# kyumcu/firedancer

Measured on AMD Instinct MI355X. Metric: Ed25519 verifies/sec, higher is better.
Workload: dtype u32

## Files before the change

firedancer_amd/csrc/fd_curve25519_dev.h:

```cpp

#ifndef FD_CURVE25519_DEV_H
#define FD_CURVE25519_DEV_H

#include "fd_f25519_dev.h"

#if defined(__HIPCC__)
#define FD_GE_FN __device__ __forceinline__
#else
#define FD_GE_FN static
#endif

struct ge_p3     { fe X, Y, Z, T; };
struct ge_cached { fe YpX, YmX, T2d, Z2; };
struct ge_precomp{ fe YpX, YmX, T2d; };

FD_FN void fe_const_d( fe & r ) {
  r.v[0]=0x35978a3u; r.v[1]=0x0d37284u; r.v[2]=0x3156ebdu; r.v[3]=0x06a0a0eu; r.v[4]=0x001c029u;
  r.v[5]=0x179e898u; r.v[6]=0x3a03cbbu; r.v[7]=0x1ce7198u; r.v[8]=0x2e2b6ffu; r.v[9]=0x1480db3u;
}
FD_FN void fe_const_d2( fe & r ) {
  r.v[0]=0x2b2f159u; r.v[1]=0x1a6e509u; r.v[2]=0x22add7au; r.v[3]=0x0d4141du; r.v[4]=0x0038052u;
  r.v[5]=0x0f3d130u; r.v[6]=0x3407977u; r.v[7]=0x19ce331u; r.v[8]=0x1c56dffu; r.v[9]=0x0901b67u;
}
FD_FN void fe_const_sqrtm1( fe & r ) {
// ... 70 lines not shown
  fe_mul( TT, p.T, q.T2d );
  FE_FENCE();
  fe_add( D, p.Z, p.Z );
  fe_sub( E, PP, MM );
  fe_add( H, PP, MM );
  fe_add( G, D, TT );
  fe_sub( F, D, TT );
  fe_mul( r.X, F, E );
  FE_FENCE();
  fe_mul( r.Y, H, G );
  FE_FENCE();
  fe_mul( r.Z, F, G );
  FE_FENCE();
  if( want_t ) fe_mul( r.T, H, E );
  FE_FENCE();
}

FD_FN void ge_to_cached( ge_cached & c, ge_p3 const & p ) {
  fe d2; fe_const_d2( d2 );
  fe_add( c.YpX, p.Y, p.X );
  fe_sub( c.YmX, p.Y, p.X );
  fe_mul( c.T2d, p.T, d2 );
  FE_FENCE();
  fe_add( c.Z2, p.Z, p.Z );
}

FD_FN void ge_from_cached( ge_p3 & r, ge_cached const & c ) {
  fe t;
  t.v[0] = c.YpX.v[0] + FE_4P0 - c.YmX.v[0];
#pragma unroll
// ... 118 lines not shown
```

firedancer_amd/csrc/fd_diag.h:

```cpp

#ifndef FD_DIAG_H
#define FD_DIAG_H

#if !defined(FD_DIAG_BUILD)
#if defined(FD_DIAG_NO_VTAB_STORE) || defined(FD_DIAG_VTAB_ONE_ENTRY) || defined(FD_DIAG_VTAB_NO_TAIL) || \
    defined(FD_DIAG_SC_TABLES) || defined(FD_DIAG_NT_TABLES) || defined(FD_DIAG_NT_INV) ||                 \
    defined(FD_DIAG_SC_INV_AFTER) || defined(FD_DIAG_COMB_POS) || defined(FD_DIAG_LSORT_TIMEOUT) ||         \
    defined(FD_DIAG_PIPE_OVERLAP) || defined(FD_DIAG_NO_HAND) || defined(FD_DIAG_NO_ARENA) || defined(FD_DIAG_STORE_COAL) || \
    defined(FD_DIAG_STORE_SMALL) || defined(FD_DIAG_STORE_COAL_NT)
#error "FD_DIAG_* builds a wrong-results diagnostic variant: only tools/build_var.sh (FD_DIAG_BUILD) may define one"
#endif
#endif


#define FD_VTAB_TAIL        1
#define FD_COMB_POS_RUN     FD_CTAB_POS
#define FD_LSORT_SPIN       (1u << 20)
#define FD_DIAG_VTAB_STORE( m, tl, w )   do {} while( 0 )
#define FD_DIAG_FETCH_ENTRY( e )         do {} while( 0 )
#define FD_DIAG_PHASE_BC_ENTRY()         do {} while( 0 )
#define FD_DIAG_AFTER_TABLES()           do {} while( 0 )
#define FD_DIAG_SCR_ORDER                1
#define FD_DIAG_NO_HAND_ON               0
#define FD_DIAG_NO_ARENA_ON              0

#if defined(__HIPCC__)
__device__ __forceinline__ uint32_t fd_diag_bp_word( int j ) { return j ? 0x66666666u : 0x66666658u; }
__device__ __forceinline__ uint32_t fd_diag_hash( uint64_t g, uint32_t j ) {
  uint32_t x = (uint32_t)g * 0x9e3779b1u ^ (j + 1u) * 0x85ebca6bu;
  x ^= x >> 15; x *= 0x2c1b3c6du; x ^= x >> 12; x *= 0x297a2d39u; x ^= x >> 15;
  return x;
}
#endif

#if defined(FD_DIAG_BUILD)

#if defined(FD_DIAG_VTAB_NO_TAIL)
#undef  FD_VTAB_TAIL
#define FD_VTAB_TAIL 0
// ... 10 lines not shown
#endif

#if defined(FD_DIAG_PIPE_OVERLAP)
#undef  FD_DIAG_SCR_ORDER
#define FD_DIAG_SCR_ORDER 0
#endif

#if defined(FD_DIAG_NO_HAND)
#undef  FD_DIAG_NO_HAND_ON
#define FD_DIAG_NO_HAND_ON 1
#endif

#if defined(FD_DIAG_NO_ARENA)
#undef  FD_DIAG_NO_ARENA_ON
#define FD_DIAG_NO_ARENA_ON 1
#endif

#if defined(FD_DIAG_VTAB_ONE_ENTRY)
#undef  FD_DIAG_FETCH_ENTRY
#define FD_DIAG_FETCH_ENTRY( e ) do { (e) = 0u; } while( 0 )
#endif

#if defined(FD_DIAG_NO_VTAB_STORE)
#undef  FD_DIAG_VTAB_STORE
#define FD_DIAG_VTAB_STORE( m, tl, w ) do {                                                       \
    if( (w)[0] == 0xdeadbeefu && (w)[1] == 0xdeadbeefu ) (m)[0] = make_uint4( (w)[2], (w)[3], (w)[4], (w)[5] ); \
    return; } while( 0 )
#elif defined(FD_DIAG_STORE_COAL)
#undef  FD_DIAG_VTAB_STORE
#define FD_DIAG_VTAB_STORE( m, tl, w ) do {                                                       \
// ... 68 lines not shown
```

firedancer_amd/csrc/fd_ed25519_gpu_host.cpp:

```cpp

#include <hip/hip_runtime_api.h>
#include <dlfcn.h>
#include <stdlib.h>
#include <string.h>
#include <stdio.h>
#include <time.h>
#include <condition_variable>
#include <functional>
#include <thread>
#include <mutex>
#include <string>
#include <unordered_map>
#include <vector>

#include "fd_ed25519_gpu_abi.h"
#include "fd_diag.h"

static uint64_t align_up( uint64_t x, uint64_t a ) { return (x + a - 1u) / a * a; }

static unsigned char const fd_ed25519_gpu_hsaco[] = {
#include "fd_ed25519_gpu_hsaco.inc"
};
#include "fd_build_id.h"

// ... 909 lines not shown
    if( s->phand[k] ) hipFree( s->phand[k] );
    if( s->pst[k] )   hipFree( s->pst[k] );
    if( s->pnw[k] )   hipFree( s->pnw[k] );
    s->phand[k] = NULL; s->pst[k] = NULL; s->pnw[k] = NULL;
  }
  for( int k=0; k<2; k++ ) {
    if( s->pacc[k] )  hipFree( s->pacc[k] );
    if( s->pcode[k] ) hipFree( s->pcode[k] );
    s->pacc[k] = NULL; s->pcode[k] = NULL;
  }
  if( s->perr ) hipHostFree( s->perr );
  s->pvtab = NULL; s->perr = NULL; s->d_perr = NULL;
  s->pipe_ready = 0;
}

static int
pipe_reserve( fd_dev_state * s ) {
  if( s->pipe_ready ) return FD_ED25519_GPU_OK;
  HIPCK( hipSetDevice( s->dev ) );
  pipe_free( s );
  uint64_t cap = s->sig_cap;
  uint64_t words = (uint64_t)FD_VTAB_N * FD_VTAB_WORDS * (2u * FD_PIPE_SETS * cap);
  int err = FD_ED25519_GPU_OK;
  if( fd_gpu_test_fail_alloc() || hipMalloc( &s->pvtab, (words + FD_VTAB_WORDS) * sizeof(uint32_t) ) != hipSuccess ) {
    s->pvtab = NULL; err = FD_ED25519_GPU_ERR_OOM;
  }
  for( int k=0; k<FD_PIPE_SETS && !err; k++ ) {
    if( hipMalloc( &s->phand[k], (uint64_t)FD_PH_WORDS * cap * sizeof(uint32_t) ) != hipSuccess ) { s->phand[k] = NULL; err = FD_ED25519_GPU_ERR_OOM; break; }
    if( hipMalloc( &s->pst[k], cap ) != hipSuccess )               { s->pst[k] = NULL; err = FD_ED25519_GPU_ERR_OOM; break; }
    if( hipMalloc( &s->pnw[k], cap / 64u + 1u ) != hipSuccess )    { s->pnw[k] = NULL; err = FD_ED25519_GPU_ERR_OOM; break; }
// ... 2 lines not shown
    if( fd_gpu_test_fail_alloc() ||
        hipMalloc( &s->pacc[k], (uint64_t)FD_PACC_WORDS * cap * sizeof(uint32_t) ) != hipSuccess ) { s->pacc[k] = NULL; err = FD_ED25519_GPU_ERR_OOM; break; }
    if( hipMalloc( &s->pcode[k], cap ) != hipSuccess ) { s->pcode[k] = NULL; err = FD_ED25519_GPU_ERR_OOM; break; }
  }
  if( !err && (hipHostMalloc( (void **)&s->perr, FD_PIPE_ERR_RING * sizeof(uint32_t), hipHostMallocMapped ) != hipSuccess ||
               hipHostGetDevicePointer( (void **)&s->d_perr, s->perr, 0 ) != hipSuccess) ) {
    if( s->perr ) hipHostFree( s->perr );
    s->perr = NULL; s->d_perr = NULL; err = FD_ED25519_GPU_ERR_OOM;
  }
  if( !err ) {
    for( int k=0; k<FD_PIPE_ERR_RING; k++ ) ((volatile uint32_t *)s->perr)[ k ] = 0u;
    err = vtab_id_fill( s, s->pvtab, 2u * FD_PIPE_SETS * cap );
  }
  if( err ) { pipe_free( s ); return err; }
  s->pctr = 0; s->pb[0].n = 0; s->pb[1].n = 0; s->pb[0].tag = -1; s->pb[1].tag = -1;
  char const * e = getenv( "FD_ED25519_GPU_PIPE_KB" );
  long kb = e ? atol( e ) : 8;
  s->pkb = kb < 1 ? 1u : (uint64_t)kb;
  e = getenv( "FD_ED25519_GPU_PIPE_LSORT" );
  s->plsort = !(e && e[0] == '0');
  e = getenv( "FD_ED25519_GPU_PIPE_PRIO" );
  s->pprio = 0;
  if( e && strlen( e ) == 3 )
    for( int k=0; k<3; k++ ) s->pprio |= (uint64_t)((e[k] - '0') & 3) << (2*k);
  s->pipe_ready = 1;
  return FD_ED25519_GPU_OK;
}

static int
pipe_launch( fd_ed25519_gpu_t * ctx, fd_dev_state * s, uint8_t const * d_arena, uint64_t arena_sz,
             fd_ed25519_desc_t const * d_desc, uint64_t n, uint32_t const * d_ncnt, int8_t * d_out, int tag,
             hipStream_t st, int * done_tag, uint32_t const * kpre = NULL, fparse_args const * fp = NULL ) {
  pipe_args a;
  memset( &a, 0, sizeof(a) );
// ... 115 lines not shown
  int err2 = scr_release( s, st );
  return err ? err : err2;
}

int
fd_ed25519_gpu_pipe_flush_dev( fd_ed25519_gpu_t * ctx, int dev_idx, void * stream ) {
  if( !ctx || dev_idx < 0 || dev_idx >= ctx->ndev ) return FD_ED25519_GPU_ERR_ARG;
  fd_dev_state * s = &ctx->d[ dev_idx ];
  if( !s->pipe_ready ) return FD_ED25519_GPU_OK;
  if( ctx->aq_cnt || ctx->fq_cnt ) return FD_ED25519_GPU_ERR_BUSY;
  for( int k=0; k<2 && pipe_busy( s ); k++ ) {
    int err = fd_ed25519_gpu_pipe_dev( ctx, dev_idx, NULL, 0u, NULL, 0u, NULL, stream );
    if( err ) return err;
  }
  return FD_ED25519_GPU_OK;
}

int
fd_ed25519_gpu_pipe_status( fd_ed25519_gpu_t * ctx, int dev_idx ) {
  if( !ctx || dev_idx < 0 || dev_idx >= ctx->ndev ) return FD_ED25519_GPU_ERR_ARG;
  return pipe_err_take( &ctx->d[ dev_idx ] );
}


static int
aslot_reserve( fd_dev_state * s, fd_dev_state::aslot * e, uint64_t span_sz, uint64_t m ) {
  if( !e->copied ) {
    if( hipEventCreateWithFlags( &e->copied, s->evflags ) != hipSuccess ) { e->copied = NULL; return FD_ED25519_GPU_ERR_LAUNCH; }
    if( hipEventCreateWithFlags( &e->done, s->doneflags ) != hipSuccess ) {
      hipEventDestroy( e->copied ); e->copied = NULL; e->done = NULL; return FD_ED25519_GPU_ERR_LAUNCH;
// ... 1059 lines not shown
```

firedancer_amd/csrc/fd_ed25519_gpu_kern.hip:

```cpp

#include <hip/hip_runtime.h>

#include "fd_ed25519_gpu_abi.h"
#include "fd_f25519_dev.h"
#include "fd_curve25519_dev.h"
#include "fd_sha512_dev.h"
#include "fd_sha256_dev.h"
#include "fd_scalar_dev.h"
#include "fd_lattice_dev.h"
#include "fd_diag.h"

#ifndef FD_OPT_FIRSTWIN
#define FD_OPT_FIRSTWIN 1
#endif
#ifndef FD_OPT_COMBCHK
#define FD_OPT_COMBCHK 1
#endif
#ifndef FD_OPT_IDROW
#define FD_OPT_IDROW 2
#endif
#ifndef FD_OPT_TAIL1
#define FD_OPT_TAIL1 1
#endif
#ifndef FD_OPT_APARSE
#define FD_OPT_APARSE 1
#endif
#ifndef FD_OPT_APRIO
#define FD_OPT_APRIO 1
#endif
#ifndef FD_OPT_BNOT
#define FD_OPT_BNOT 1
#endif
#ifndef FD_OPT_X4
#define FD_OPT_X4 1
#endif

#ifdef FD_PHASE_STAMPS
#define FD_NSTAMP 8
#define FD_TL_BASE 8
#define FD_STAMP_WORDS_DEV (8u + 4096u * 12u * 4u)
#define STAMP( i ) do { FE_FENCE(); if( _st ) _st[ i ] = __builtin_amdgcn_s_memtime(); FE_FENCE(); } while( 0 )
#else
#define STAMP( i ) do {} while( 0 )
#endif


typedef unsigned int fd_u4a4 __attribute__(( ext_vector_type( 4 ), aligned( 4 ) ));

template<int M>
// ... 204 lines not shown
      int k = 4*j + i;
      w[i] = (k == FD_VW( 0, 0 ) || k == FD_VW( 1, 0 )) ? 1u : (k == FD_VW( 3, 0 ) ? 2u : 0u);
    }
    m[j] = make_uint4( w[0], w[1], w[2], w[3] );
  }
  tl[0] = make_uint4( 0u, 0u, 0u, 0u ); tl[1] = make_uint4( 0u, 0u, 0u, 0u );
}

__device__ __forceinline__ uint32_t vtab_entry( uint32_t db ) {
  uint32_t e;
  asm( "v_sad_u32 %0, %1, 8, 0" : "=v"(e) : "v"(db) );
  return min( e, 8u );
}

__device__ __forceinline__ void vtab_store( uint32_t * vtab, uint64_t cap, uint64_t t, int e, ge_cached const & c,
                                            bool tail = true ) {
  uint32_t w[ 40 ];
#pragma unroll
  for( int j=0; j<10; j++ ) {
    w[FD_VW(0,j)] = c.YpX.v[j]; w[FD_VW(1,j)] = c.YmX.v[j]; w[FD_VW(2,j)] = c.T2d.v[j]; w[FD_VW(3,j)] = c.Z2.v[j];
  }
  uint4 const * mc; uint4 const * tc;
  vtab_ptrs( vtab, cap, t, (uint32_t)e, &mc, &tc );
  uint4 * m = (uint4 *)mc; uint4 * tl = (uint4 *)tc;
  FD_DIAG_VTAB_STORE( m, tl, w );
#pragma unroll
  for( int j=0; j<8; j++ ) m[j] = make_uint4( w[4*j], w[4*j+1], w[4*j+2], w[4*j+3] );
#if FD_VTAB_TAIL
  if( tail ) {
#pragma unroll
    for( int j=0; j<2; j++ ) tl[j] = make_uint4( w[32+4*j], w[33+4*j], w[34+4*j], w[35+4*j] );
  }
#endif
}

__device__ __forceinline__ void vtab_build( uint32_t * vtab, uint64_t cap, uint64_t t, ge_p3 const & Q ) {
  ge_p3 nQ = Q;
  { fe x; fe_neg( x, Q.X ); fe_carry( nQ.X, x ); fe_neg( x, Q.T ); fe_carry( nQ.T, x ); }
  ge_cached c;
// ... 149 lines not shown
#ifdef FD_PHASE_STAMPS
                                                     , uint64_t * _st
#endif
                                                     , uint32_t const * krow = nullptr
                                                     ) {
  uint32_t k[ 8 ];
  if( krow ) {
    uint4 k0 = ((uint4 const *)krow)[0], k1 = ((uint4 const *)krow)[1];
    k[0] = k0.x; k[1] = k0.y; k[2] = k0.z; k[3] = k0.w; k[4] = k1.x; k[5] = k1.y; k[6] = k1.z; k[7] = k1.w;
  } else {
    hash_ram<FASTBLK>( k, sig, pub, args.arena, d.msg_off, d.msg_sz, lim_dw );
  }
  FE_FENCE();
  STAMP( 2 );
  lat_short_vector( k, u, v, un );
  FE_FENCE();
  uint32_t pr[ 16 ];
#pragma unroll
  for( int j=0; j<16; j++ ) pr[j] = 0u;
#pragma unroll
  for( int i=0; i<8; i++ ) {
    uint64_t c = 0;
#pragma unroll
    for( int j=0; j<8; j++ ) { uint64_t t = (uint64_t)v[i] * sig[8+j] + pr[i+j] + c; pr[i+j] = (uint32_t)t; c = t >> 32; }
    pr[i+8] = (uint32_t)c;
  }
  sc_reduce512( w, pr );
  *nbits = max( bitlen8( u ), bitlen8( v ) );
}

// ... 221 lines not shown
    {
      dma_wait();
      uint32_t w[ 40 ];
      lds_entry_words<10>( w, buf, lane, dbr < 8u );
      if( i > lo ) dba = ydig_p( yu, lane, i-1, nw, wn, uneg );
      FE_FENCE();
      if( i > lo ) vtab_fetch_lds( buf, vtab, cap, ta, dba );
      lds_entry_finish( q, w, dbr < 8u );
    }
    FE_FENCE();
    ge_add_cached( acc, acc, q, i == lo && last_t );
    FE_FENCE();
  }
}

__device__ __forceinline__ void comb_lds( ge_p3 & acc, uint4 * buf, uint32_t const * yw, int lane, uint32_t const * ctab ) {
#define FD_WDIG( k ) comb_digit_w( yw[ ((23*(k)) >> 5)*64 + lane ], ((23*(k)) >> 5) < 7 ? yw[ (((23*(k)) >> 5) + 1)*64 + lane ] : 0u, (k) )
  int d = FD_WDIG( 0 );
  ctab_fetch_lds( buf, ctab, 0, d );
#pragma unroll 1
  for( int k=0; k<FD_COMB_POS_RUN; k++ ) {
    ge_precomp bp;
    {
      dma_wait();
      uint32_t w[ 32 ];
      lds_words<8>( w, buf, lane );
      int dn = k + 1 < FD_COMB_POS_RUN ? FD_WDIG( k + 1 ) : 0;
      FE_FENCE();
      if( k + 1 < FD_COMB_POS_RUN ) ctab_fetch_lds( buf, ctab, k + 1, dn );
      ctab_finish( bp, w, d );
// ... 482 lines not shown
  uint64_t m_uneg = __ballot( (ps & FD_PIPE_ST_UNEG) != 0 );
  uint64_t m_desc = __ballot( (ps & FD_PIPE_ST_DESC) != 0 ), m_bads = __ballot( (ps & FD_PIPE_ST_BADS) != 0 );
  if( !__ballot( valid ) ) return;
  int code;
  if( phb ) {
    bool desc_ok = (m_desc >> lane) & 1u, bad_s = (m_bads >> lane) & 1u;
    int stA = 0, stR = 0;
    if( desc_ok && !bad_s ) {
      uint32_t enc[ 8 ];
#pragma unroll
      for( int j=0; j<8; j++ ) enc[j] = FD_DIAG_NO_HAND_ON ? fd_diag_bp_word( j ) : hand[ (uint64_t)(FD_PH_A + j)*cap + gid ];
      ge_p3 Q;
      int sm;
      int ok = ge_decode_small( Q, enc, !args.ref_codes, &sm );
      FE_FENCE();
      if( ok && !sm ) vtab_build( args.vtab, vcap, (2u*set)*cap + gid, Q );
      stA = (ok ? 1 : 0) | (sm ? 2 : 0);
      FE_FENCE();
    }
    uint64_t m_aok = __ballot( (stA & 1) != 0 ), m_asm = __ballot( (stA & 2) != 0 );
    uint64_t gr = gid;
    asm volatile( "" : "+v"(gr) );
    if( desc_ok && !bad_s ) {
      uint32_t enc[ 8 ];
#pragma unroll
      for( int j=0; j<8; j++ ) enc[j] = FD_DIAG_NO_HAND_ON ? fd_diag_bp_word( j ) : hand[ (uint64_t)(FD_PH_R + j)*cap + gr ];
      ge_p3 Q;
      int sm;
      int ok = ge_decode_small( Q, enc, !args.ref_codes, &sm );
      FE_FENCE();
      bool aok = (m_aok >> lane) & 1u, asm_ = (m_asm >> lane) & 1u;
      if( ok && !sm && aok && !asm_ ) vtab_build( args.vtab, vcap, (2u*set + 1u)*cap + gid, Q );
      stR = (ok ? 1 : 0) | (sm ? 2 : 0);
      FE_FENCE();
    }
    stA = (int)((m_aok >> lane) & 1u) | (int)(((m_asm >> lane) & 1u) << 1);
    FD_DIAG_AFTER_TABLES();
    code = verify_precode( args, desc_ok, bad_s, stA, stR );
    if( valid && !FD_DIAG_NO_HAND_ON ) a.code_b[ gid ] = (int8_t)code;
  } else {
    code = valid && !FD_DIAG_NO_HAND_ON ? (int)a.code_c[ gid ] : 0;
  }
  bool run = valid && code == 0;
  int P = __builtin_amdgcn_readfirstlane( (int)(phb ? a.nw_b : a.nw_c)[ gid >> 6 ] );
  int nw = ((P + 3) >> 2) + 1, wn = P - 4*(nw - 2);
  int split = max( nw - (int)a.kb, 0 );
  int hi = phb ? nw : split, lo = phb ? split : 0;
  ge_p3 acc;
  if( run ) {
    hand_to_lds( y, hand, cap, gid, lane, FD_PH_YU, phb ? 16 : 24 );
    if( phb || FD_DIAG_NO_HAND_ON ) ge_identity( acc );
    else {
      uint32_t const * o = a.acc_c + gid;
#pragma unroll
      for( int j=0; j<10; j++ ) {
        acc.X.v[j] = o[ (uint64_t)j*cap ]; acc.Y.v[j] = o[ (uint64_t)(10+j)*cap ];
        acc.Z.v[j] = o[ (uint64_t)(20+j)*cap ];
        if( !FD_OPT_BNOT ) acc.T.v[j] = o[ (uint64_t)(30+j)*cap ];
      }
    }
    FE_FENCE();
    if( hi > lo )
      chain_seg( acc, buf, y, y + 8*64, lane, ((m_uneg >> lane) & 1u) != 0, args.vtab, vcap,
                 (2u*set)*cap + gid, (2u*set + 1u)*cap + gid, nw, hi, lo, wn, !(FD_OPT_BNOT && phb) );
    FE_FENCE();
    if( phb ) {
      uint32_t * o = a.acc_b + gid;
#if FD_DIAG_NO_HAND_ON
      uint32_t sink = 0u;
#pragma unroll
      for( int j=0; j<10; j++ ) sink ^= acc.X.v[j] ^ acc.Y.v[j] ^ acc.Z.v[j] ^ (FD_OPT_BNOT ? 0u : acc.T.v[j]);
      if( sink == 0xdeadbeefu && acc.X.v[0] == 0xdeadbeefu ) o[ 0 ] = sink;
#else
#pragma unroll
      for( int j=0; j<10; j++ ) {
        o[ (uint64_t)j*cap ] = acc.X.v[j]; o[ (uint64_t)(10+j)*cap ] = acc.Y.v[j];
        o[ (uint64_t)(20+j)*cap ] = acc.Z.v[j];
        if( !FD_OPT_BNOT ) o[ (uint64_t)(30+j)*cap ] = acc.T.v[j];
      }
#endif
    } else {
#if FD_OPT_COMBCHK
      int eq = comb_lds_eq( acc, buf, y + 16*64, lane, args.ctab );
#else
      comb_lds( acc, buf, y + 16*64, lane, args.ctab );
      fe dl;
      int ex = fe_is_zero( acc.X );
      fe_sub( dl, acc.Y, acc.Z ); fe_carry( dl, dl );
      int eq = ex & fe_is_zero( dl );
#endif
      code = eq ? FD_ED25519_SUCCESS : FD_ED25519_ERR_MSG;
    }
  }
// ... 679 lines not shown
```

firedancer_amd/ed25519.py:

```python
import collections
import ctypes
import os

import numpy as np

QUEUE_DEPTH = 5
STAGE_DEPTH = 8

FD_ED25519_SUCCESS = 0
FD_ED25519_ERR_SIG = -1
FD_ED25519_ERR_PUBKEY = -2
FD_ED25519_ERR_MSG = -3
CODE_BAD_DESC = -128

GPU_OK = 0
GPU_PENDING = 1

CODES_AVX512 = 0
CODES_REF = 1

SHA_MSG_DTYPE = np.dtype([("off", "<u4"), ("sz", "<u4")])

PRECOMPILE_DTYPE = np.dtype([("data_off", "<u4"), ("data_sz", "<u4"), ("txn_instr_lo", "<u4"),
                             ("txn_instr_cnt", "<u4")])
# ... 45 lines not shown
    lib.fd_ed25519_gpu_poll.argtypes = [vp]
    lib.fd_ed25519_gpu_poll_block.argtypes = [vp]
    lib.fd_ed25519_gpu_pending.argtypes = [vp]
    lib.fd_ed25519_gpu_pipe_status.argtypes = [vp, i32]
    lib.fd_ed25519_gpu_host_stats.argtypes = [vp, vp, i32]
    lib.fd_ed25519_gpu_test_ctab_stats.argtypes = [i32, vp, vp]
    lib.fd_ed25519_gpu_launch_stats.argtypes = [vp, vp, vp]
    lib.fd_ed25519_gpu_build_id.restype = ctypes.c_char_p
    lib.fd_ed25519_gpu_build_id.argtypes = []
    lib.fd_ed25519_gpu_runtime.restype = ctypes.c_char_p
    lib.fd_ed25519_gpu_runtime.argtypes = []
    lib.fd_ed25519_gpu_host_is_registered.argtypes = [vp, u64]
    lib.fd_ed25519_verify_batch_gpu_dev.argtypes = [vp, i32, vp, u64, vp, u64, vp, vp]
    lib.fd_ed25519_gpu_pipe_dev.argtypes = [vp, i32, vp, u64, vp, u64, vp, vp]
    lib.fd_ed25519_gpu_pipe_flush_dev.argtypes = [vp, i32, vp]
    lib.fd_ed25519_gpu_verify.argtypes = [vp, ctypes.c_char_p, u64, ctypes.c_char_p, ctypes.c_char_p,
                                          ctypes.POINTER(ctypes.c_int)]
    lib.fd_ed25519_gpu_verify_batch_single_msg.argtypes = [vp, ctypes.c_char_p, u64, ctypes.c_char_p,
                                                           ctypes.c_char_p, u64, ctypes.POINTER(ctypes.c_int)]
    lib.fd_ed25519_gpu_txn_reduce.restype = ctypes.c_int64
    lib.fd_ed25519_gpu_txn_reduce.argtypes = [vp, vp, u64, vp, u64]
    lib.fd_ed25519_gpu_test_lattice.argtypes = [vp, vp, u64, vp]
    lib.fd_ed25519_gpu_test_field.argtypes = [vp, ctypes.c_int, vp, vp, u64, vp]
    lib.fd_sha512_batch_gpu.argtypes = [vp, vp, u64, vp, u64, vp]
    lib.fd_sha512_batch_gpu_dev.argtypes = [vp, i32, vp, u64, vp, u64, vp, vp]
    lib.fd_sha256_batch_gpu.argtypes = [vp, vp, u64, vp, u64, vp]
    lib.fd_sha256_batch_gpu_dev.argtypes = [vp, i32, vp, u64, vp, u64, vp, vp]
    lib.fd_ed25519_gpu_sign_batch.argtypes = [vp, vp, u64, vp, u64, vp]
    lib.fd_ed25519_gpu_sign_batch_dev.argtypes = [vp, i32, vp, u64, vp, u64, vp, vp]
    lib.fd_ed25519_gpu_public_from_private_batch.argtypes = [vp, vp, u64, vp]
# ... 264 lines not shown
        r = self.lib.fd_ed25519_verify_batch_gpu_dev(self.ctx, dev_idx, d_arena, arena_sz, d_desc, desc_cnt,
                                                     d_out, stream)
        if r:
            raise GpuError("fd_ed25519_verify_batch_gpu_dev: %s (%d)" % (strerror(r), r))

    def pipe_dev(self, d_arena, arena_sz, d_desc, desc_cnt, d_out, stream=0, dev_idx=0):
        r = self.lib.fd_ed25519_gpu_pipe_dev(self.ctx, dev_idx, d_arena, arena_sz, d_desc, desc_cnt, d_out, stream)
        if r:
            raise GpuError("fd_ed25519_gpu_pipe_dev: %s (%d)" % (strerror(r), r))

    def pipe_flush_dev(self, stream=0, dev_idx=0):
        r = self.lib.fd_ed25519_gpu_pipe_flush_dev(self.ctx, dev_idx, stream)
        if r:
            raise GpuError("fd_ed25519_gpu_pipe_flush_dev: %s (%d)" % (strerror(r), r))

    def verify(self, msg, sig, pub):
        out = ctypes.c_int(0)
        r = self.lib.fd_ed25519_gpu_verify(self.ctx, msg, len(msg), sig, pub, ctypes.byref(out))
        if r:
            raise GpuError(strerror(r))
        return out.value

    def verify_batch_single_msg(self, msg, sigs, pubs, n):
        out = ctypes.c_int(0)
        r = self.lib.fd_ed25519_gpu_verify_batch_single_msg(self.ctx, msg, len(msg), sigs or b"\0" * 64,
                                                            pubs or b"\0" * 32, n, ctypes.byref(out))
        if r:
            raise GpuError(strerror(r))
        return out.value

# ... 140 lines not shown
```

include/fd_ed25519_gpu.h:

```cpp

#ifndef FD_ED25519_GPU_H
#define FD_ED25519_GPU_H

#include <stddef.h>
#include <stdint.h>

#ifdef __cplusplus
extern "C" {
#endif

#define FD_ED25519_SUCCESS     ( 0)
#define FD_ED25519_ERR_SIG     (-1)
#define FD_ED25519_ERR_PUBKEY  (-2)
#define FD_ED25519_ERR_MSG     (-3)

#define FD_ED25519_GPU_CODE_BAD_DESC (-128)

#define FD_ED25519_GPU_QUEUE_DEPTH 5

#define FD_ED25519_GPU_STAGE_DEPTH 8

#define FD_ED25519_GPU_OK          (0)
#define FD_ED25519_GPU_PENDING     (1)
#define FD_ED25519_GPU_ERR_NODEV   (-100)
// ... 51 lines not shown
int fd_ed25519_gpu_poll( fd_ed25519_gpu_t * ctx );
int fd_ed25519_gpu_poll_block( fd_ed25519_gpu_t * ctx );
int fd_ed25519_gpu_pending( fd_ed25519_gpu_t const * ctx );

int fd_ed25519_verify_batch_gpu_dev( fd_ed25519_gpu_t * ctx, int dev_idx,
                                     uint8_t const * d_arena, uint64_t arena_sz,
                                     fd_ed25519_desc_t const * d_desc, uint64_t desc_cnt,
                                     int8_t * d_out, void * stream );

int fd_ed25519_gpu_pipe_dev( fd_ed25519_gpu_t * ctx, int dev_idx,
                             uint8_t const * d_arena, uint64_t arena_sz,
                             fd_ed25519_desc_t const * d_desc, uint64_t desc_cnt,
                             int8_t * d_out, void * stream );
int fd_ed25519_gpu_pipe_flush_dev( fd_ed25519_gpu_t * ctx, int dev_idx, void * stream );
int fd_ed25519_gpu_pipe_status( fd_ed25519_gpu_t * ctx, int dev_idx );

int fd_ed25519_gpu_verify( fd_ed25519_gpu_t * ctx, uint8_t const * msg, uint64_t msg_sz,
                           uint8_t const sig[ 64 ], uint8_t const pub[ 32 ], int * out );
int fd_ed25519_gpu_verify_batch_single_msg( fd_ed25519_gpu_t * ctx, uint8_t const * msg, uint64_t msg_sz,
                                            uint8_t const * sigs, uint8_t const * pubs, uint64_t n, int * out );

int64_t fd_ed25519_gpu_txn_reduce( int8_t const * out_code, fd_ed25519_desc_t const * desc, uint64_t n,
                                   int8_t * out_txn_code, uint64_t out_cap );

char const * fd_ed25519_gpu_strerror( int err );

char const * fd_ed25519_gpu_build_id( void );

char const * fd_ed25519_gpu_runtime( void );

// ... 179 lines not shown
```

Baseline: 126.3 million.

## Use joint two-scalar precomputed table for A and R in verification chain

Replaces the two separate per-point window tables for A and R with a single joint table indexed by a combined digit pair. Entries hold small linear combinations of A and R, built using shared add/sub formulas that reuse intermediate products. The main chain then does one cached addition per half-window instead of two separate additions. This cuts point additions and table fetches in the hot loop, at the cost of a more complex table build, extra parking of state in LDS, and a different memory layout for the table. It also adds a pipe_kb query API, caps the pipe KB env value, and adds a diagnostic flag for the lattice fallback.

```diff
diff --git a/firedancer_amd/csrc/fd_curve25519_dev.h b/firedancer_amd/csrc/fd_curve25519_dev.h
--- a/firedancer_amd/csrc/fd_curve25519_dev.h
+++ b/firedancer_amd/csrc/fd_curve25519_dev.h
@@ -108,6 +108,65 @@
   FE_FENCE();
   if( want_t ) fe_mul( r.T, H, E );
   FE_FENCE();
+}
+
+struct ge_addsub_st { fe G, F, Z; };
+FD_GE_FN void ge_addsub_sum( ge_p3 & s, ge_addsub_st & st, ge_p3 const & p, ge_cached const & q, int dm ) {
+  fe a, b, PP, MM, TT, D, E, H;
+  fe_add( a, p.Y, p.X );
+  fe_sub( b, p.Y, p.X );
+  fe_mul( PP, a, q.YpX );
+  FE_FENCE();
+  fe_mul( MM, b, q.YmX );
+  FE_FENCE();
+  fe_mul( TT, p.T, q.T2d );
+  FE_FENCE();
+  if( dm == 0 ) { fe_mul( D, p.Z, q.Z2 ); FE_FENCE(); }
+  else if( dm == 1 ) fe_add( D, p.Z, p.Z );
+  else if( dm == 2 ) D = q.Z2;
+  else { fe_set0( D ); D.v[0] = 2u; }
+  fe_add( st.G, D, TT );
+  fe_sub( st.F, D, TT );
+  fe_sub( E, PP, MM );
+  fe_add( H, PP, MM );
+  fe_mul( s.X, st.F, E );
+  FE_FENCE();
+  fe_mul( s.Y, H, st.G );
+  FE_FENCE();
+  fe_mul( s.Z, st.F, st.G );
+  FE_FENCE();
+  fe_mul( s.T, H, E );
+  FE_FENCE();
+  st.Z = s.Z;
+}
+FD_GE_FN void ge_addsub_diff( ge_p3 & d, ge_addsub_st const & st, ge_p3 const & p, ge_cached const & q, bool rev ) {
+  fe a, b, PQ, MQ, E, H;
+  fe_add( a, p.Y, p.X );
+  fe_sub( b, p.Y, p.X );
+  fe_mul( PQ, a, q.YmX );
+  FE_FENCE();
+  fe_mul( MQ, b, q.YpX );
+  FE_FENCE();
+  if( rev ) fe_sub( E, MQ, PQ ); else fe_sub( E, PQ, MQ );
+  fe_add( H, PQ, MQ );
+  fe_mul( d.X, E, st.G );
+  FE_FENCE();
+  fe_mul( d.Y, st.F, H );
+  FE_FENCE();
+  d.Z = st.Z;
+  fe_mul( d.T, H, E );
+  FE_FENCE();
+}
+
+FD_FN void ge_xyz_from_cached( ge_p3 & r, ge_cached const & c ) {
+  fe t;
+  t.v[0] = c.YpX.v[0] + FE_4P0 - c.YmX.v[0];
+#pragma unroll
+  for( int i=1; i<10; i++ ) t.v[i] = c.YpX.v[i] + ((i&1) ? FE_4PO : FE_4PE) - c.YmX.v[i];
+  fe_carry( r.X, t );
+  fe_add( t, c.YpX, c.YmX );
+  fe_carry( r.Y, t );
+  fe_carry( r.Z, c.Z2 );
 }
 
 FD_FN void ge_to_cached( ge_cached & c, ge_p3 const & p ) {
diff --git a/firedancer_amd/csrc/fd_diag.h b/firedancer_amd/csrc/fd_diag.h
--- a/firedancer_amd/csrc/fd_diag.h
+++ b/firedancer_amd/csrc/fd_diag.h
@@ -7,7 +7,7 @@
     defined(FD_DIAG_SC_TABLES) || defined(FD_DIAG_NT_TABLES) || defined(FD_DIAG_NT_INV) ||                 \
     defined(FD_DIAG_SC_INV_AFTER) || defined(FD_DIAG_COMB_POS) || defined(FD_DIAG_LSORT_TIMEOUT) ||         \
     defined(FD_DIAG_PIPE_OVERLAP) || defined(FD_DIAG_NO_HAND) || defined(FD_DIAG_NO_ARENA) || defined(FD_DIAG_STORE_COAL) || \
-    defined(FD_DIAG_STORE_SMALL) || defined(FD_DIAG_STORE_COAL_NT)
+    defined(FD_DIAG_STORE_SMALL) || defined(FD_DIAG_STORE_COAL_NT) || defined(FD_DIAG_LAT_FALLBACK)
 #error "FD_DIAG_* builds a wrong-results diagnostic variant: only tools/build_var.sh (FD_DIAG_BUILD) may define one"
 #endif
 #endif
@@ -23,6 +23,7 @@
 #define FD_DIAG_SCR_ORDER                1
 #define FD_DIAG_NO_HAND_ON               0
 #define FD_DIAG_NO_ARENA_ON              0
+#define FD_DIAG_LAT_FALLBACK_ON          0
 
 #if defined(__HIPCC__)
 __device__ __forceinline__ uint32_t fd_diag_bp_word( int j ) { return j ? 0x66666666u : 0x66666658u; }
@@ -63,6 +64,11 @@
 #if defined(FD_DIAG_NO_ARENA)
 #undef  FD_DIAG_NO_ARENA_ON
 #define FD_DIAG_NO_ARENA_ON 1
+#endif
+
+#if defined(FD_DIAG_LAT_FALLBACK)
+#undef  FD_DIAG_LAT_FALLBACK_ON
+#define FD_DIAG_LAT_FALLBACK_ON 1
 #endif
 
 #if defined(FD_DIAG_VTAB_ONE_ENTRY)
diff --git a/firedancer_amd/csrc/fd_ed25519_gpu_host.cpp b/firedancer_amd/csrc/fd_ed25519_gpu_host.cpp
--- a/firedancer_amd/csrc/fd_ed25519_gpu_host.cpp
+++ b/firedancer_amd/csrc/fd_ed25519_gpu_host.cpp
@@ -947,6 +947,14 @@
   s->pipe_ready = 0;
 }
 
+#define FD_PIPE_KB_MAX 31
+static uint64_t
+pipe_kb_env( void ) {
+  char const * e = getenv( "FD_ED25519_GPU_PIPE_KB" );
+  long kb = e ? atol( e ) : 8;
+  return kb < 1 ? 1u : (kb > FD_PIPE_KB_MAX ? (uint64_t)FD_PIPE_KB_MAX : (uint64_t)kb);
+}
+
 static int
 pipe_reserve( fd_dev_state * s ) {
   if( s->pipe_ready ) return FD_ED25519_GPU_OK;
@@ -979,10 +987,8 @@
   }
   if( err ) { pipe_free( s ); return err; }
   s->pctr = 0; s->pb[0].n = 0; s->pb[1].n = 0; s->pb[0].tag = -1; s->pb[1].tag = -1;
-  char const * e = getenv( "FD_ED25519_GPU_PIPE_KB" );
-  long kb = e ? atol( e ) : 8;
-  s->pkb = kb < 1 ? 1u : (uint64_t)kb;
-  e = getenv( "FD_ED25519_GPU_PIPE_LSORT" );
+  s->pkb = pipe_kb_env();
+  char const * e = getenv( "FD_ED25519_GPU_PIPE_LSORT" );
   s->plsort = !(e && e[0] == '0');
   e = getenv( "FD_ED25519_GPU_PIPE_PRIO" );
   s->pprio = 0;
@@ -1128,6 +1134,13 @@
     if( err ) return err;
   }
   return FD_ED25519_GPU_OK;
+}
+
+int
+fd_ed25519_gpu_pipe_kb( fd_ed25519_gpu_t const * ctx, int dev_idx ) {
+  if( !ctx || dev_idx < 0 || dev_idx >= ctx->ndev ) return FD_ED25519_GPU_ERR_ARG;
+  fd_dev_state const * s = &ctx->d[ dev_idx ];
+  return (int)(s->pipe_ready ? s->pkb : pipe_kb_env());
 }
 
 int
diff --git a/firedancer_amd/csrc/fd_ed25519_gpu_kern.hip b/firedancer_amd/csrc/fd_ed25519_gpu_kern.hip
--- a/firedancer_amd/csrc/fd_ed25519_gpu_kern.hip
+++ b/firedancer_amd/csrc/fd_ed25519_gpu_kern.hip
@@ -8,6 +8,7 @@
 #include "fd_sha256_dev.h"
 #include "fd_scalar_dev.h"
 #include "fd_lattice_dev.h"
+#include "fd_joint2_dev.h"
 #include "fd_diag.h"
 
 #ifndef FD_OPT_FIRSTWIN
@@ -33,6 +34,9 @@
 #endif
 #ifndef FD_OPT_X4
 #define FD_OPT_X4 1
+#endif
+#ifndef FD_OPT_JOINT2
+#define FD_OPT_JOINT2 1
 #endif
 
 #ifdef FD_PHASE_STAMPS
@@ -267,7 +271,7 @@
 }
 
 __device__ __forceinline__ void vtab_store( uint32_t * vtab, uint64_t cap, uint64_t t, int e, ge_cached const & c,
-                                            bool tail = true ) {
+                                            bool tail = true, bool joint = false  ) {
   uint32_t w[ 40 ];
 #pragma unroll
   for( int j=0; j<10; j++ ) {
@@ -276,6 +280,7 @@
   uint4 const * mc; uint4 const * tc;
   vtab_ptrs( vtab, cap, t, (uint32_t)e, &mc, &tc );
   uint4 * m = (uint4 *)mc; uint4 * tl = (uint4 *)tc;
+  if( joint ) tl = (uint4 *)((uint32_t *)tl + (uint64_t)FD_VTAB_N * cap * 32u);
   FD_DIAG_VTAB_STORE( m, tl, w );
 #pragma unroll
   for( int j=0; j<8; j++ ) m[j] = make_uint4( w[4*j], w[4*j+1], w[4*j+2], w[4*j+3] );
@@ -455,6 +460,11 @@
   FE_FENCE();
   STAMP( 2 );
   lat_short_vector( k, u, v, un );
+  if( FD_DIAG_LAT_FALLBACK_ON ) {
+#pragma unroll
+    for( int j=0; j<8; j++ ) { u[j] = k[j]; v[j] = j ? 0u : 1u; }
+    *un = 0;
+  }
   FE_FENCE();
   uint32_t pr[ 16 ];
 #pragma unroll
@@ -706,6 +716,174 @@
   }
 }
 
+
+
+__device__ __forceinline__ void vtab_ptrs_j2( uint32_t const * vtab, uint64_t cap, uint64_t t, uint32_t e,
+                                              uint4 const ** m, uint4 const ** tl ) {
+  vtab_ptrs( vtab, cap, t, e, m, tl );
+  *tl = (uint4 const *)((uint32_t const *)*tl + (uint64_t)FD_VTAB_N * cap * 32u);
+}
+
+__device__ __forceinline__ void vtab_load( ge_cached & c, uint32_t const * vtab, uint64_t cap, uint64_t t, uint32_t row, bool z2 ) {
+  asm volatile( "" : "+v"(t) );
+  uint4 const * m; uint4 const * tl;
+  vtab_ptrs_j2( vtab, cap, t, row, &m, &tl );
+  uint32_t w[ 40 ];
+#pragma unroll
+  for( int j=0; j<8; j++ ) { uint4 v = m[j]; w[4*j] = v.x; w[4*j+1] = v.y; w[4*j+2] = v.z; w[4*j+3] = v.w; }
+#pragma unroll
+  for( int j=0; j<2; j++ ) {
+    uint4 v = z2 ? tl[j] : make_uint4( 0u, 0u, 0u, 0u );
+    w[32+4*j] = v.x; w[33+4*j] = v.y; w[34+4*j] = v.z; w[35+4*j] = v.w;
+  }
+#pragma unroll
+  for( int j=0; j<10; j++ ) {
+    c.YpX.v[j] = w[FD_VW(0,j)]; c.YmX.v[j] = w[FD_VW(1,j)]; c.T2d.v[j] = w[FD_VW(2,j)]; c.Z2.v[j] = w[FD_VW(3,j)];
+  }
+}
+
+#define FD_J2_STORE( e, c, tail ) vtab_store( vtab, cap, t, e, c, tail, true )
+
+__device__ __forceinline__ void vtab_store_j2( uint32_t * vtab, uint64_t cap, uint64_t t, int e, ge_p3 const & p ) {
+  ge_cached c;
+  ge_to_cached( c, p ); FD_J2_STORE( e, c, true );
+  FE_FENCE();
+}
+
+__device__ __forceinline__ void vtab_dbl_j2( uint32_t * vtab, uint64_t cap, uint64_t t, int e2, int e ) {
+  ge_cached c;
+  vtab_load( c, vtab, cap, t, e, true );
+  ge_p3 P;
+  ge_xyz_from_cached( P, c );
+  FE_FENCE();
+  ge_dbl( P, P, true );
+  vtab_store_j2( vtab, cap, t, e2, P );
+}
+
+__device__ __forceinline__ void vtab_build_j2_a( uint32_t * vtab, uint64_t cap, uint64_t t, ge_p3 const & Q ) {
+  ge_p3 nQ = Q;
+  { fe x; fe_neg( x, Q.X ); fe_carry( nQ.X, x ); fe_neg( x, Q.T ); fe_carry( nQ.T, x ); }
+  ge_cached c;
+  ge_to_cached( c, nQ ); FD_J2_STORE( 5, c, true );
+  ge_p3 P;
+  ge_dbl( P, nQ, true ); vtab_store_j2( vtab, cap, t, 10, P );
+}
+
+__device__ __forceinline__ void j2_park( uint32_t * park, int lane, ge_p3 const & p ) {
+#pragma unroll
+  for( int j=0; j<10; j++ ) { park[ j*64 + lane ] = p.X.v[j]; park[ (10+j)*64 + lane ] = p.Y.v[j]; park[ (20+j)*64 + lane ] = p.T.v[j]; }
+}
+__device__ __forceinline__ void j2_unpark( ge_p3 & p, uint32_t const * park, int lane ) {
+  asm volatile( "" : "+v"(lane) );
+#pragma unroll
+  for( int j=0; j<10; j++ ) { p.X.v[j] = park[ j*64 + lane ]; p.Y.v[j] = park[ (10+j)*64 + lane ]; p.T.v[j] = park[ (20+j)*64 + lane ]; }
+  fe_set1( p.Z );
+}
+
+__device__ __forceinline__ void vtab_build_j2( uint32_t * vtab, uint64_t cap, uint64_t t, ge_p3 const & Q, uint32_t * park, int lane ) {
+  ge_cached c;
+  ge_p3 nR, s;
+  ge_addsub_st st;
+  {
+    nR = Q;
+    fe x; fe_neg( x, Q.X ); fe_carry( nR.X, x ); fe_neg( x, Q.T ); fe_carry( nR.T, x );
+    j2_park( park, lane, nR );
+    ge_to_cached( c, nR ); FD_J2_STORE( 1, c, !(FD_OPT_IDROW == 2 && FD_OPT_TAIL1) );
+    FE_FENCE();
+  }
+  vtab_load( c, vtab, cap, t, 5, false );  j2_unpark( nR, park, lane );
+  ge_addsub_sum( s, st, nR, c, 3 );        vtab_store_j2( vtab, cap, t, 6, s );
+  vtab_load( c, vtab, cap, t, 5, false );  j2_unpark( nR, park, lane );
+  ge_addsub_diff( s, st, nR, c, true );    vtab_store_j2( vtab, cap, t, 4, s );
+  vtab_load( c, vtab, cap, t, 10, true );  j2_unpark( nR, park, lane );
+  ge_addsub_sum( s, st, nR, c, 2 );        vtab_store_j2( vtab, cap, t, 11, s );
+  vtab_load( c, vtab, cap, t, 10, false ); j2_unpark( nR, park, lane );
+  ge_addsub_diff( s, st, nR, c, true );    vtab_store_j2( vtab, cap, t, 9, s );
+  ge_p3 P;
+  j2_unpark( nR, park, lane );
+  ge_dbl( P, nR, true );                   vtab_store_j2( vtab, cap, t, 2, P );
+  vtab_load( c, vtab, cap, t, 5, false );
+  ge_addsub_sum( s, st, P, c, 1 );         vtab_store_j2( vtab, cap, t, 7, s );
+  ge_addsub_diff( s, st, P, c, true );     vtab_store_j2( vtab, cap, t, 3, s );
+  vtab_dbl_j2( vtab, cap, t, 12, 6 );
+  vtab_dbl_j2( vtab, cap, t, 8, 4 );
+}
+#undef FD_J2_STORE
+
+__device__ __forceinline__ uint32_t j2_code( uint32_t xu, uint32_t xv, int part, int single ) {
+  uint32_t sh = part ? 2u : 0u, wd = (part || single) ? 3u : 2u;
+  return 5u * __builtin_amdgcn_ubfe( xu, sh, wd ) + __builtin_amdgcn_ubfe( xv, sh, wd );
+}
+
+__device__ __forceinline__ void vtab_fetch_lds_j2( uint4 * buf, uint32_t const * vtab, uint64_t cap, uint64_t t, uint32_t c ) {
+  uint32_t e;
+  asm( "v_sad_u32 %0, %1, 12, 0" : "=v"(e) : "v"(c) );
+  e = min( e, 12u );
+  FD_DIAG_FETCH_ENTRY( e );
+  uint4 const * m; uint4 const * tl;
+  vtab_ptrs_j2( vtab, cap, t, e, &m, &tl );
+  glds_record<8>( m, buf );
+#if FD_VTAB_TAIL
+  glds_record<2>( tl, buf + 64*8 );
+#endif
+}
+
+__device__ __forceinline__ void chain_seg_j2( ge_p3 & acc, uint4 * buf, uint32_t const * yu, uint32_t const * yv, int lane,
+                                              bool uneg, uint32_t const * vtab, uint64_t cap, uint64_t t,
+                                              int nw, int hi, int lo, int wn, bool last_t = true ) {
+  int s = 2*hi - 1, send = 2*lo;
+  if( !fd_j2_exists( s, nw, wn ) ) s--;
+#define FD_J2_DIGITS( i ) do {                                                                                 \
+    uint32_t xb = ((i) == nw-2 && wn <= 2) ? 2u - 8u : 2u;                                                     \
+    xu = ydig_p( yu, lane, (i), nw, wn, uneg ) + xb; xv = ydig_p( yv, lane, (i), nw, wn, false ) + xb;         \
+  } while( 0 )
+  uint32_t xu, xv;
+  FD_J2_DIGITS( s >> 1 );
+  uint32_t sel = j2_code( xu, xv, s & 1, (s >> 1) == nw-2 && wn <= 2 );
+  vtab_fetch_lds_j2( buf, vtab, cap, t, sel );
+#define FD_J2_TAKE( q ) do {                                                                                  \
+    dma_wait();                                                                                                \
+    uint32_t w[ 40 ];                                                                                          \
+    bool neg = sel < 12u;                                                                                      \
+    lds_entry_words<10>( w, buf, lane, neg );                                                                  \
+    uint32_t seln = 12u;                                                                                       \
+    if( sn >= send ) {                                                                                         \
+      if( (sn >> 1) != (s >> 1) ) FD_J2_DIGITS( sn >> 1 );                                                     \
+      seln = j2_code( xu, xv, sn & 1, (sn >> 1) == nw-2 && wn <= 2 );                                          \
+    }                                                                                                          \
+    FE_FENCE();                                                                                                \
+    if( sn >= send ) vtab_fetch_lds_j2( buf, vtab, cap, t, seln );    \
+    lds_entry_finish( (q), w, neg );                                                                           \
+    sel = seln;                                                                                                \
+  } while( 0 )
+#if FD_OPT_FIRSTWIN
+  if( hi == nw ) {
+    int sn = fd_j2_next( s, nw, wn );
+    ge_cached q;
+    FD_J2_TAKE( q );
+    FE_FENCE();
+    ge_from_cached( acc, q );
+    FE_FENCE();
+    s = sn;
+  }
+#endif
+#pragma unroll 1
+  while( s >= send ) {
+    int nd = fd_j2_dbl( s, nw, wn );
+    if( nd == 2 ) { ge_dbl( acc, acc, false ); FE_FENCE(); }
+    if( nd >= 1 ) { ge_dbl( acc, acc, true ); FE_FENCE(); }
+    int sn = fd_j2_next( s, nw, wn );
+    ge_cached q;
+    FD_J2_TAKE( q );
+    FE_FENCE();
+    ge_add_cached( acc, acc, q, s == send && last_t );
+    FE_FENCE();
+    s = sn;
+  }
+#undef FD_J2_TAKE
+#undef FD_J2_DIGITS
+}
+
 __device__ __forceinline__ void comb_lds( ge_p3 & acc, uint4 * buf, uint32_t const * yw, int lane, uint32_t const * ctab ) {
 #define FD_WDIG( k ) comb_digit_w( yw[ ((23*(k)) >> 5)*64 + lane ], ((23*(k)) >> 5) < 7 ? yw[ (((23*(k)) >> 5) + 1)*64 + lane ] : 0u, (k) )
   int d = FD_WDIG( 0 );
@@ -1218,7 +1396,11 @@
       int sm;
       int ok = ge_decode_small( Q, enc, !args.ref_codes, &sm );
       FE_FENCE();
+#if FD_OPT_JOINT2
+      if( ok && !sm ) vtab_build_j2_a( args.vtab, vcap >> 1, set*cap + gid, Q );
+#else
       if( ok && !sm ) vtab_build( args.vtab, vcap, (2u*set)*cap + gid, Q );
+#endif
       stA = (ok ? 1 : 0) | (sm ? 2 : 0);
       FE_FENCE();
     }
@@ -1234,7 +1416,11 @@
       int ok = ge_decode_small( Q, enc, !args.ref_codes, &sm );
       FE_FENCE();
       bool aok = (m_aok >> lane) & 1u, asm_ = (m_asm >> lane) & 1u;
+#if FD_OPT_JOINT2
+      if( ok && !sm && aok && !asm_ ) vtab_build_j2( args.vtab, vcap >> 1, set*cap + gr, Q, (uint32_t *)buf, lane );
+#else
       if( ok && !sm && aok && !asm_ ) vtab_build( args.vtab, vcap, (2u*set + 1u)*cap + gid, Q );
+#endif
       stR = (ok ? 1 : 0) | (sm ? 2 : 0);
       FE_FENCE();
     }
@@ -1250,6 +1436,7 @@
   int nw = ((P + 3) >> 2) + 1, wn = P - 4*(nw - 2);
   int split = max( nw - (int)a.kb, 0 );
   int hi = phb ? nw : split, lo = phb ? split : 0;
+  bool hand_t = !FD_OPT_BNOT || split == 0;
   ge_p3 acc;
   if( run ) {
     hand_to_lds( y, hand, cap, gid, lane, FD_PH_YU, phb ? 16 : 24 );
@@ -1260,13 +1447,18 @@
       for( int j=0; j<10; j++ ) {
         acc.X.v[j] = o[ (uint64_t)j*cap ]; acc.Y.v[j] = o[ (uint64_t)(10+j)*cap ];
         acc.Z.v[j] = o[ (uint64_t)(20+j)*cap ];
-        if( !FD_OPT_BNOT ) acc.T.v[j] = o[ (uint64_t)(30+j)*cap ];
+        if( hand_t ) acc.T.v[j] = o[ (uint64_t)(30+j)*cap ];
       }
     }
     FE_FENCE();
     if( hi > lo )
+#if FD_OPT_JOINT2
+      chain_seg_j2( acc, buf, y, y + 8*64, lane, ((m_uneg >> lane) & 1u) != 0, args.vtab, vcap >> 1, set*cap + gid,
+                    nw, hi, lo, wn, !phb || hand_t );
+#else
       chain_seg( acc, buf, y, y + 8*64, lane, ((m_uneg >> lane) & 1u) != 0, args.vtab, vcap,
-                 (2u*set)*cap + gid, (2u*set + 1u)*cap + gid, nw, hi, lo, wn, !(FD_OPT_BNOT && phb) );
+                 (2u*set)*cap + gid, (2u*set + 1u)*cap + gid, nw, hi, lo, wn, !phb || hand_t );
+#endif
     FE_FENCE();
     if( phb ) {
       uint32_t * o = a.acc_b + gid;
@@ -1280,7 +1472,7 @@
       for( int j=0; j<10; j++ ) {
         o[ (uint64_t)j*cap ] = acc.X.v[j]; o[ (uint64_t)(10+j)*cap ] = acc.Y.v[j];
         o[ (uint64_t)(20+j)*cap ] = acc.Z.v[j];
-        if( !FD_OPT_BNOT ) o[ (uint64_t)(30+j)*cap ] = acc.T.v[j];
+        if( hand_t ) o[ (uint64_t)(30+j)*cap ] = acc.T.v[j];
       }
 #endif
     } else {
diff --git a/firedancer_amd/csrc/fd_joint2_dev.h b/firedancer_amd/csrc/fd_joint2_dev.h
--- /dev/null
+++ b/firedancer_amd/csrc/fd_joint2_dev.h
@@ -0,0 +1,59 @@
+
+#ifndef FD_JOINT2_DEV_H
+#define FD_JOINT2_DEV_H
+
+#include <stdint.h>
+
+#if defined(__HIPCC__)
+#define FD_J2_FN __device__ __forceinline__
+#else
+#define FD_J2_FN static inline
+#endif
+
+#define FD_J2_CLASSES 12
+
+FD_J2_FN uint32_t fd_j2_half_x( uint32_t x, int part, int single ) {
+  uint32_t sh = part ? 2u : 0u, wd = (part || single) ? 3u : 2u;
+#if defined(__HIP_DEVICE_COMPILE__)
+  return __builtin_amdgcn_ubfe( x, sh, wd );
+#else
+  return (x >> sh) & ((1u << wd) - 1u);
+#endif
+}
+FD_J2_FN uint32_t fd_j2_x( uint32_t db, int single ) { return db + (single ? 2u - 8u : 2u); }
+FD_J2_FN uint32_t fd_j2_half_b( uint32_t db, int part, int single ) { return fd_j2_half_x( fd_j2_x( db, single ), part, single ); }
+FD_J2_FN int fd_j2_half( uint32_t db, int part, int single ) { return (int)fd_j2_half_b( db, part, single ) - 2; }
+
+FD_J2_FN int fd_j2_exists( int s, int nw, int wn ) {
+  return s >= 0 && s < 2*nw && !(s == 2*(nw-2) + 1 && wn <= 2);
+}
+FD_J2_FN int fd_j2_next( int s, int nw, int wn ) {
+  return (s - 1 == 2*(nw-2) + 1 && wn <= 2) ? s - 2 : s - 1;
+}
+FD_J2_FN int fd_j2_shift( int s, int nw, int wn ) {
+  int i = s >> 1, part = s & 1;
+  return (i == nw-1 ? 4*(nw-2) + wn : 4*i) + 2*part;
+}
+FD_J2_FN int fd_j2_dbl( int s, int nw, int wn ) {
+  int i = s >> 1, part = s & 1;
+  if( i == nw-1 ) return part ? 0 : 2;
+  if( i == nw-2 ) return part ? wn - 2 : (wn <= 2 ? wn : 2);
+  return 2;
+}
+FD_J2_FN int fd_j2_count( int nw, int wn ) { return 2*nw - (wn <= 2 ? 1 : 0); }
+
+FD_J2_FN uint32_t fd_j2_class( int i, int j, int * lead_neg ) {
+  uint32_t c = (uint32_t)(5*(i + 2) + (j + 2));
+  *lead_neg = c < 12u;
+  return (c < 12u ? 12u - c : c - 12u) - 1u;
+}
+
+FD_J2_FN uint32_t fd_j2_code( uint32_t bi, uint32_t bj ) { return 5u*bi + bj; }
+FD_J2_FN uint32_t fd_j2_entry_b( uint32_t bi, uint32_t bj, int * neg ) {
+  uint32_t c = fd_j2_code( bi, bj );
+  *neg = c < 12u;
+  return c < 12u ? 12u - c : c - 12u;
+}
+FD_J2_FN uint32_t fd_j2_entry( int i, int j, int * neg ) { return fd_j2_entry_b( (uint32_t)(i + 2), (uint32_t)(j + 2), neg ); }
+
+#endif
diff --git a/firedancer_amd/ed25519.py b/firedancer_amd/ed25519.py
--- a/firedancer_amd/ed25519.py
+++ b/firedancer_amd/ed25519.py
@@ -83,6 +83,7 @@
     lib.fd_ed25519_verify_batch_gpu_dev.argtypes = [vp, i32, vp, u64, vp, u64, vp, vp]
     lib.fd_ed25519_gpu_pipe_dev.argtypes = [vp, i32, vp, u64, vp, u64, vp, vp]
     lib.fd_ed25519_gpu_pipe_flush_dev.argtypes = [vp, i32, vp]
+    lib.fd_ed25519_gpu_pipe_kb.argtypes = [vp, i32]
     lib.fd_ed25519_gpu_verify.argtypes = [vp, ctypes.c_char_p, u64, ctypes.c_char_p, ctypes.c_char_p,
                                           ctypes.POINTER(ctypes.c_int)]
     lib.fd_ed25519_gpu_verify_batch_single_msg.argtypes = [vp, ctypes.c_char_p, u64, ctypes.c_char_p,
@@ -377,6 +378,12 @@
         if r:
             raise GpuError("fd_ed25519_gpu_pipe_flush_dev: %s (%d)" % (strerror(r), r))
 
+    def pipe_kb(self, dev_idx=0):
+        r = self.lib.fd_ed25519_gpu_pipe_kb(self.ctx, dev_idx)
+        if r < 0:
+            raise GpuError("fd_ed25519_gpu_pipe_kb: %s (%d)" % (strerror(r), r))
+        return r
+
     def verify(self, msg, sig, pub):
         out = ctypes.c_int(0)
         r = self.lib.fd_ed25519_gpu_verify(self.ctx, msg, len(msg), sig, pub, ctypes.byref(out))
diff --git a/include/fd_ed25519_gpu.h b/include/fd_ed25519_gpu.h
--- a/include/fd_ed25519_gpu.h
+++ b/include/fd_ed25519_gpu.h
@@ -89,6 +89,7 @@
                              int8_t * d_out, void * stream );
 int fd_ed25519_gpu_pipe_flush_dev( fd_ed25519_gpu_t * ctx, int dev_idx, void * stream );
 int fd_ed25519_gpu_pipe_status( fd_ed25519_gpu_t * ctx, int dev_idx );
+int fd_ed25519_gpu_pipe_kb( fd_ed25519_gpu_t const * ctx, int dev_idx );
 
 int fd_ed25519_gpu_verify( fd_ed25519_gpu_t * ctx, uint8_t const * msg, uint64_t msg_sz,
                            uint8_t const sig[ 64 ], uint8_t const pub[ 32 ], int * out );
```

New measurement: 127.2 million, median of 6. About the same (+0.8%).
